# RuihanGao/visual-tactile-synthesis

Hardware: AMD Instinct MI355X
Metric: train_images_per_sec (higher is better)
Workload: dtype f32; 1 GPU; skitG G+D1+D2 train step, 1024x1024 sketch->(RGB,tactile), 4 images/GPU, 64 tactile patches/image, LPIPS/CLIP terms off (no weights offline); global_batch=4, parallelism=dp1, losses_finite=True, hip_graph=True, d2_visualisation_pass=True, train_only=False, full=False

## Files before the change

### include/vts.h

```cpp
#ifndef VTS_H
#define VTS_H

#include <stdint.h>

#ifdef __cplusplus
extern "C" {
#endif

#define VTS_OK 0
#define VTS_ERR_ARG (-1)
#define VTS_ERR_UNSUPPORTED (-2)
#define VTS_ERR_LAUNCH (-3)

#define VTS_ACT_NONE 0
#define VTS_ACT_LRELU 1
#define VTS_ACT_RELU 2
#define VTS_ACT_TANH 3

const char* vts_last_error(void);
const char* vts_last_kernel(void);
int vts_version(void);
int vts_capture_node_count(void* stream, int* nodes, int* kernel_nodes);

typedef struct vts_operand {
  const float* data;
  const float* scale;
  const float* shift;
  int C;
  int64_t nstride;
} vts_operand;

typedef struct vts_conv_desc {
  vts_operand in0, in1;
  int N, IH, IW, OH, OW, Cout;
  int stride, pad, transposed;
  const float* w;
  int ws_co, ws_ci;
  const float* bias;
  float* out;
  int64_t out_nstride;
  int act_in, act_out;
  vts_operand dmask;
  int dmask_act;
  int accumulate;
  float* ws;
  int64_t ws_floats;
  int pad_dx;
} vts_conv_desc;

int64_t vts_conv4x4_ws_floats(const vts_conv_desc* d);

int vts_conv4x4(const vts_conv_desc* d, void* stream);

typedef struct vts_wgrad_desc {
  vts_operand lo0, lo1, hi0, hi1;
  int act_lo, act_hi;
  int N, LH, LW, HH, HW;
  int stride, pad;
  float* dw;
  int accumulate;
  int pad_dx;
  int defer;
} vts_wgrad_desc;

int64_t vts_wgrad4x4_ws_floats(const vts_wgrad_desc* d);
int vts_wgrad4x4(const vts_wgrad_desc* d, float* ws, void* stream);

#define VTS_REDUCE_MAX_SEG 4
typedef struct vts_reduce_job {
  float* dw;
  int64_t nel;
  int accumulate;
  int nseg;
  const float* part[VTS_REDUCE_MAX_SEG];
  int pw[VTS_REDUCE_MAX_SEG];
} vts_reduce_job;
int vts_wgrad_reduce_batch(const vts_reduce_job* jobs , int njobs, void* stream);

int vts_channel_sum(const float* x, int64_t nstride, int N, int C, int HW, float* out, int accumulate,
                    float* ws, int* counters , void* stream);
int64_t vts_channel_sum_ws_floats(int N, int C, int HW);

typedef struct vts_norm_desc {
  const float* x;
  int64_t nstride;
  int N, C, HW;
  int mode;
  float eps, momentum;
  const float* gamma;
  const float* beta;
  float* running_mean;
  float* running_var;
  int64_t* num_batches_tracked;
  float* scale;
  float* shift;
  float* mean_out;
  float* rstd_out;
  int* counters;
  int ngroups;
  int gstart[9];
  float* stat_mean_out;
  float* stat_uvar_out;
  const float* ext_mean;
  const float* ext_uvar;
  int ext_after;
// ... 391 lines not shown
```

### visual-tactile-synthesis_amd/csrc/vts_conv.hip

```cpp
#include "vts_conv_kernel.h"

thread_local int t_stat_spl = 0;

namespace {

__global__ __launch_bounds__(256) void conv_split_epilogue_kernel(const ConvK p, int KS) {
  const int co = blockIdx.y, n = blockIdx.z;
  const int64_t oplane = (int64_t)p.OH * p.OW;
  const int64_t o = (int64_t)blockIdx.x * 256 + threadIdx.x;
  if (o >= oplane) return;
  float v = 0.f;
  for (int ks = 0; ks < KS; ++ks) v += p.part[(((int64_t)ks * p.N + n) * p.Cout + co) * oplane + o];
  v += p.bias ? p.bias[co] : 0.f;
  if (p.act_out == VTS_ACT_TANH) v = tanhf(v);
  if (p.dm) {
    const float dsc = p.dmsc ? p.dmsc[n * p.dmC + co] : 1.f, dsh = p.dmsh ? p.dmsh[n * p.dmC + co] : 0.f;
    v *= vts_act_grad(p.dm[n * p.dmns + co * oplane + o] * dsc + dsh, p.dm_act);
  }
  float* ob = p.out + n * p.ons + co * oplane + o;
  *ob = p.accumulate ? *ob + v : v;
}

struct InStatsOut {
  float *scale, *shift, *mean, *rstd;
  float eps;
};
__global__ __launch_bounds__(256) void conv_split_epilogue_in_kernel(const ConvK p, int KS, const InStatsOut q) {
  __shared__ float red[16];
  const int g = blockIdx.x, n = g / p.Cout, co = g - n * p.Cout;
  const int HW = p.OH * p.OW;
  const float bias = p.bias ? p.bias[co] : 0.f;
  float v[16];
#pragma unroll
  for (int e = 0; e < 16; ++e) {
    const int o = e * 256 + threadIdx.x;
    float a = 0.f;
    if (o < HW) {
      for (int ks = 0; ks < KS; ++ks) a += p.part[(((int64_t)ks * p.N + n) * p.Cout + co) * HW + o];
      a += bias;
      p.out[n * p.ons + (int64_t)co * HW + o] = a;
    }
    v[e] = a;
  }
  const float cnt = (float)HW;
  float s = 0.f;
#pragma unroll
  for (int e = 0; e < 16; ++e) s += v[e];
  const float mean = block_sum(s, red) / cnt;
  float m2 = 0.f;
#pragma unroll
  for (int e = 0; e < 16; ++e) {
    const float d = v[e] - mean;
    if (e * 256 + (int)threadIdx.x < HW) m2 += d * d;
  }
  m2 = block_sum(m2, red);
// ... 18 lines not shown
#pragma unroll
  for (int e = 0; e < 16; ++e) {
    const int o = e * 256 + threadIdx.x;
    float a = 0.f, t = 0.f;
    if (o < HW) {
      for (int ks = 0; ks < KS; ++ks) a += p.part[(((int64_t)ks * p.N + n) * p.Cout + co) * HW + o];
      a += bias;
      t = dmb[o] * dsc + dsh;
      a *= vts_act_grad(t, p.dm_act);
      if (p.accumulate) a += ob[o];
    }
    v[e] = a;
    tn[e] = t;
  }
  float s1 = 0.f, s2 = 0.f;
#pragma unroll
  for (int e = 0; e < 16; ++e) {
    s1 += v[e];
    s2 = fmaf(v[e], tn[e], s2);
  }
  s1 = block_sum(s1, red);
  s2 = block_sum(s2, red);
  const float m1 = s1 / (float)HW, m2 = s2 / (float)HW;
#pragma unroll
  for (int e = 0; e < 16; ++e) {
    const int o = e * 256 + threadIdx.x;
    if (o < HW) ob[o] = dsc * (v[e] - m1 - tn[e] * m2);
  }
}

inline void full_tile(int transposed, int stride, int nr, int& rw, int& mt) {
  static const int T[2][2][5][2] = {
      {{{2, 4}, {1, 4}, {1, 4}, {1, 2}, {1, 2}}, {{2, 4}, {1, 4}, {1, 4}, {1, 2}, {1, 2}}},
      {{{2, 4}, {1, 4}, {1, 4}, {1, 2}, {1, 2}}, {{1, 4}, {1, 2}, {1, 2}, {1, 1}, {1, 1}}}};
  rw = T[transposed][stride - 1][nr - 1][0];
  mt = T[transposed][stride - 1][nr - 1][1];
}

}

extern "C" int64_t vts_conv4x4_ws_floats(const vts_conv_desc* d) {
  if (!d) return 0;
  const int nchunks = (d->in0.C + (d->in1.data ? d->in1.C : 0) + 3) / 4;
  const int ks_max = nchunks / 2 < 1 ? 1 : (nchunks / 2 > 320 ? 320 : nchunks / 2);
  return (int64_t)ks_max * d->N * d->Cout * d->OH * d->OW;
}

struct StatWs {
  float* p;
  int64_t floats;
};
static int conv4x4_impl(const vts_conv_desc* d, void* stream, const vts_norm_desc* nd, int* fused, StatWs sw, bool bsums = false, bool in_bwd_ok = false);
int vts_norm_finalize_partials(const vts_norm_desc* d, const float* part, int spl, hipStream_t st);

extern "C" int vts_conv4x4(const vts_conv_desc* d, void* stream) { return conv4x4_impl(d, stream, nullptr, nullptr, StatWs{nullptr, 0}); }

extern "C" int vts_conv4x4_in(const vts_conv_desc* d, const vts_norm_desc* nd, int* fused, void* stream) {
  VTS_CHECK_ARG(nd && fused && nd->scale && nd->shift && nd->mode == 0, "vts_conv4x4_in: InstanceNorm descriptor with scale / shift outputs required");
  *fused = 0;
  return conv4x4_impl(d, stream, nd, fused, StatWs{nullptr, 0});
}

extern "C" int64_t vts_conv4x4_norm_ws_floats(const vts_conv_desc* d) {
  if (!d) return 0;
  const bool ph4 = d->transposed && d->stride == 2;
  const int GH = ph4 ? (d->OH + 1) / 2 : d->OH, GW = ph4 ? (d->OW + 1) / 2 : d->OW;
  return (int64_t)d->N * d->Cout * 3 * 4 * cdiv(GH, 4) * cdiv(GW, 16);
}

extern "C" int vts_conv4x4_norm(const vts_conv_desc* d, const vts_norm_desc* nd, float* stat_ws, int64_t stat_ws_floats, int* fused, void* stream) {
  VTS_CHECK_ARG(nd && fused && nd->scale && nd->shift && (nd->mode == 0 || nd->mode == 1), "vts_conv4x4_norm: norm descriptor with scale / shift outputs required");
  *fused = 0;
  return conv4x4_impl(d, stream, nd, fused, StatWs{stat_ws, stat_ws_floats});
}

extern "C" int vts_conv4x4_bsums(const vts_conv_desc* d, float* part, int64_t part_floats, int* slots, void* stream) {
  VTS_CHECK_ARG(d && slots && part, "vts_conv4x4_bsums: null pointer");
  const bool in_bwd_ok = *slots == -1;
  *slots = 0;
  int fused = 0;
  const int rc = conv4x4_impl(d, stream, nullptr, &fused, StatWs{part, part_floats}, true, in_bwd_ok);
  if (rc == VTS_OK && fused >= 2) *slots = fused - 2;
  if (rc == VTS_OK && fused == -1) *slots = -1;
  return rc;
}

extern "C" int vts_norm_stats_from_partials(const vts_norm_desc* nd, const float* part, int slots, void* stream) {
  return vts_norm_finalize_partials(nd, part, slots, (hipStream_t)stream);
}

static int dispatch_full(const vts_conv_desc* d, const ConvK& k, int nr, int N, hipStream_t st);

static int conv4x4_impl(const vts_conv_desc* d, void* stream, const vts_norm_desc* nd, int* fused, StatWs sw, bool bsums, bool in_bwd_ok) {
  VTS_CHECK_ARG(d && d->in0.data && d->w && d->out, "vts_conv4x4: null pointer");
  VTS_CHECK_ARG(d->stride == 1 || d->stride == 2, "vts_conv4x4: stride %d unsupported", d->stride);
  VTS_CHECK_ARG(d->Cout >= 1, "vts_conv4x4: Cout %d", d->Cout);
  if (d->Cout > 80) {
    for (int c0 = 0; c0 < d->Cout; c0 += 80) {
      vts_conv_desc g = *d;
      const int64_t oplane = (int64_t)d->OH * d->OW;
      g.Cout = d->Cout - c0 < 80 ? d->Cout - c0 : 80;
      g.w = d->w + (int64_t)c0 * d->ws_co;
      g.bias = d->bias ? d->bias + c0 : nullptr;
      g.out = d->out + c0 * oplane;
      if (d->dmask.data) {
        g.dmask.data = d->dmask.data + c0 * oplane;
        g.dmask.scale = d->dmask.scale ? d->dmask.scale + c0 : nullptr;
        g.dmask.shift = d->dmask.shift ? d->dmask.shift + c0 : nullptr;
      }
      const int rc = conv4x4_impl(&g, stream, nullptr, nullptr, StatWs{nullptr, 0});
      if (rc != VTS_OK) return rc;
    }
    return VTS_OK;
  }
  VTS_CHECK_ARG(d->N >= 1 && d->IH >= 1 && d->IW >= 1 && d->OH >= 1 && d->OW >= 1, "vts_conv4x4: bad shape");
  VTS_CHECK_ARG(d->in0.C >= 1 && d->in1.C >= 0, "vts_conv4x4: bad channel counts");
  VTS_CHECK_ARG(d->OH <= d->IH * d->stride + 16 && d->OW <= d->IW * d->stride + 16 && d->pad >= -8 && d->pad <= 8,
                "vts_conv4x4: output %dx%d / pad %d implausible for input %dx%d s%d", d->OH, d->OW, d->pad, d->IH, d->IW, d->stride);
  VTS_CHECK_ARG(d->pad_dx >= -8 && d->pad_dx <= 8 && !(d->transposed && d->stride == 2 && d->pad_dx != 0), "vts_conv4x4: bad pad_dx %d", d->pad_dx);
  if (d->transposed && d->stride == 2) {
    VTS_CHECK_ARG((d->OH + 2 * d->pad - 4) / d->stride + 1 == d->IH && (d->OW + 2 * d->pad - 4) / d->stride + 1 == d->IW && d->pad >= 0,
                  "vts_conv4x4: transposed output %dx%d inconsistent with input %dx%d s%d p%d", d->OH, d->OW, d->IH,
                  d->IW, d->stride, d->pad);
  }
  {
    const int rh0 = vts_conv_head_try(d, (hipStream_t)stream);
    if (rh0 != VTS_ERR_UNSUPPORTED) return rh0;
    static const int use_small = vts_tune_set("VTS_NO_SMALL") ? 0 : 1;
    if (use_small) {
      const int rc = vts_conv_small_try(d, (hipStream_t)stream);
      if (rc != VTS_ERR_UNSUPPORTED) return rc;
    }
  }
  ConvK k;
  k.s0 = d->in0.data; k.sc0 = d->in0.scale; k.sh0 = d->in0.shift; k.ns0 = d->in0.nstride; k.C0 = d->in0.C;
  k.s1 = d->in1.data; k.sc1 = d->in1.scale; k.sh1 = d->in1.shift; k.ns1 = d->in1.nstride;
  k.C1 = d->in1.data ? d->in1.C : 0;
  k.Cin = k.C0 + k.C1;
  k.IH = d->IH; k.IW = d->IW; k.OH = d->OH; k.OW = d->OW; k.Cout = d->Cout; k.pad = d->pad; k.padx = d->pad + d->pad_dx;
  k.w = d->w; k.ws_co = d->ws_co; k.ws_ci = d->ws_ci; k.bias = d->bias;
  k.out = d->out; k.ons = d->out_nstride;
  k.act_in = d->act_in; k.act_out = d->act_out;
  k.dm = d->dmask.data; k.dmsc = d->dmask.scale; k.dmsh = d->dmask.shift; k.dmns = d->dmask.nstride;
  k.dm_act = d->dmask_act; k.dmC = d->dmask.C;
  k.accumulate = d->accumulate;
  k.N = d->N; k.CG = 1; k.cps = 1 << 30; k.part = nullptr; k.tiles_x = 0; k.stat_part = nullptr; k.stat_spl = 0; k.bsum_part = nullptr;
#ifdef VTS_PROFILING
  static const int ablate = vts_tune("VTS_ABLATE", 0);
  k.ablate = ablate;
  k.trace = nullptr;
#endif
  k.xcd_swizzle = 1;
  static const int direct_epi = vts_tune("VTS_DIRECT_EPI", 1);
  k.direct_epi = direct_epi && (int64_t)d->Cout * d->OH * d->OW * 4 < (int64_t)OOB_OFF && (!d->dmask.data || (int64_t)d->dmask.C * d->OH * d->OW * 4 < (int64_t)OOB_OFF);
  k.ident = vts_ident();
  VTS_CHECK_ARG(k.ident, "vts_conv4x4: could not allocate the identity constants");
  {
    const int64_t wfl = (int64_t)(d->Cout - 1) * d->ws_co + (int64_t)(k.Cin - 1) * d->ws_ci + 16;
    VTS_CHECK_ARG(wfl * 4 < (int64_t)OOB_OFF && (int64_t)d->IH * d->IW * 4 < (int64_t)OOB_OFF, "vts_conv4x4: tensor too large for 30-bit buffer offsets");
    k.wbytes = (int)(wfl * 4);
  }
  k.slope_in = vts_slope(d->act_in);
  k.identity_in = (d->act_in == VTS_ACT_NONE && !d->in0.scale && !d->in0.shift && !(d->in1.data && (d->in1.scale || d->in1.shift))) ? 1 : 0;
  hipStream_t st = (hipStream_t)stream;
  const int nr = (d->Cout + 15) / 16;
  const int N = d->N;
  const bool stats_ok = nd && fused && sw.p && d->act_out == VTS_ACT_NONE && !d->dmask.data && !d->accumulate &&
                        nd->x == d->out && nd->N == N && nd->C == d->Cout && nd->HW == d->OH * d->OW && nd->nstride == d->out_nstride;
  const bool want_stats = stats_ok && k.direct_epi && sw.floats >= vts_conv4x4_norm_ws_floats(d);
  const bool bsums_ok = bsums && fused && sw.p && d->act_out == VTS_ACT_NONE && d->dmask.data;
  const bool want_bsums = bsums_ok && k.direct_epi && sw.floats >= vts_conv4x4_norm_ws_floats(d);
  {
    int spl = 0;
    const int rc = vts_conv_px_try(d, st, stats_ok ? sw.p : nullptr, (!stats_ok && bsums_ok) ? sw.p : nullptr, sw.floats, &spl);
    if (rc != VTS_ERR_UNSUPPORTED) {
      if (rc == VTS_OK && spl > 0) *fused = 2 + spl;
      return rc;
    }
    const int rt = vts_conv_thin_try(d, st);
    if (rt != VTS_ERR_UNSUPPORTED) return rt;
  }
  {
    int rw, mt;
    full_tile(d->transposed, d->stride, nr, rw, mt);
    const bool ph4 = d->transposed && d->stride == 2;
    const int GH = ph4 ? (d->OH + 1) / 2 : d->OH, GW = ph4 ? (d->OW + 1) / 2 : d->OW;
    const int full_wgs = cdiv(GW, 16 * mt) * cdiv(GH, 4 * rw) * N;
    int ck = 4;
    const int nchunks = (k.Cin + 3) / 4;
    static const int small_thr = vts_tune("VTS_SMALL_WGS", 300);
    static const int target_wgs = vts_tune("VTS_TARGET_WGS", 256);
    if (full_wgs < small_thr && (nr > 1 || nchunks >= 8)) {
      const int base = cdiv(GW, 32) * cdiv(GH, 4) * N * nr;
      int KS = target_wgs / base;
      if (KS > nchunks / 2) KS = nchunks / 2;
      if (KS < 1) KS = 1;
      int cps = cdiv(nchunks, KS);
      KS = cdiv(nchunks, cps);
      const int64_t need = (int64_t)KS * N * d->Cout * d->OH * d->OW;
      if (KS > 1 && (!d->ws || d->ws_floats < need)) { KS = 1; cps = nchunks; }
      if (k.Cin >= 32 && cps >= 4 && (cps % 2 == 0 || KS == 1)) { ck = 8; cps = (cps + 1) / 2; }
      k.CG = nr; k.cps = cps; k.part = KS > 1 ? d->ws : nullptr;
      const bool cg_stats = want_stats && KS == 1;
      if (cg_stats) k.stat_part = sw.p;
      const bool cg_bsums = want_bsums && KS == 1;
      if (cg_bsums) k.bsum_part = sw.p;
      int rc;
      if (!d->transposed) rc = d->stride == 2 ? vts_conv_split_m0s2(k, N, st, nr, KS, ck) : vts_conv_split_m0s1(k, N, st, nr, KS, ck);
      else rc = d->stride == 2 ? vts_conv_split_m1s2(k, N, st, nr, KS, ck) : vts_conv_split_m1s1(k, N, st, nr, KS, ck);
      if (rc == VTS_OK && (cg_stats || cg_bsums)) *fused = 2 + t_stat_spl;
      if (rc != VTS_OK || KS == 1) return rc;
      static const int fuse_in = vts_tune("VTS_FUSE_SPLIT_IN", 1);
      if (nd && nd->mode == 0 && fuse_in && (int64_t)d->OH * d->OW <= 4096 && d->act_out == VTS_ACT_NONE && !d->dmask.data && !d->accumulate &&
          nd->x == d->out && nd->N == N && nd->C == d->Cout && nd->HW == d->OH * d->OW && nd->nstride == d->out_nstride) {
        const InStatsOut q{nd->scale, nd->shift, nd->mean_out, nd->rstd_out, nd->eps};
        hipLaunchKernelGGL(conv_split_epilogue_in_kernel, dim3(N * d->Cout), dim3(256), 0, st, k, KS, q);
        VTS_CHECK_LAUNCH("vts_conv4x4 split epilogue + instance norm");
        vts_set_kernel("conv4x4_kernel<%d, %d, 1, 1, 2, %d, false, 0>+ksplit+in", d->transposed ? 1 : 0, d->stride, ck);
        *fused = 1;
        return VTS_OK;
      }
      if (bsums && in_bwd_ok && fused && (int64_t)d->OH * d->OW <= 4096 && d->act_out == VTS_ACT_NONE && d->dmask.data && d->dmask.scale &&
          d->dmask.shift && d->dmask.C == d->Cout) {
        hipLaunchKernelGGL(conv_split_epilogue_inbwd_kernel, dim3(N * d->Cout), dim3(256), 0, st, k, KS);
        VTS_CHECK_LAUNCH("vts_conv4x4 split epilogue + instance norm backward");
        vts_set_kernel("conv4x4_kernel<%d, %d, 1, 1, 2, %d, false, 0>+ksplit+inbwd", d->transposed ? 1 : 0, d->stride, ck);
        *fused = -1;
        return VTS_OK;
      }
      hipLaunchKernelGGL(conv_split_epilogue_kernel, dim3((unsigned)cdiv64((int64_t)d->OH * d->OW, 256), d->Cout, N), dim3(256), 0, st, k, KS);
      VTS_CHECK_LAUNCH("vts_conv4x4 split epilogue");
      return VTS_OK;
    }
  }
  if (want_stats) k.stat_part = sw.p;
  if (want_bsums) k.bsum_part = sw.p;
  const int rc = dispatch_full(d, k, nr, N, st);
  if (rc != VTS_OK || !(want_stats || want_bsums)) return rc;
  *fused = 2 + t_stat_spl;
  return VTS_OK;
}

static int dispatch_full(const vts_conv_desc* d, const ConvK& k, int nr, int N, hipStream_t st) {
  if (!d->transposed) return d->stride == 2 ? vts_conv_full_m0s2(k, nr, N, st) : vts_conv_full_m0s1(k, nr, N, st);
  return d->stride == 2 ? vts_conv_full_m1s2(k, nr, N, st) : vts_conv_full_m1s1(k, nr, N, st);
}
```

### visual-tactile-synthesis_amd/csrc/vts_conv_kernel.h

```cpp
#pragma once
#include <stdio.h>
#include <stdlib.h>
#include <string.h>

#include "vts_internal.h"

struct ConvK {
  const float *s0, *s1, *sc0, *sh0, *sc1, *sh1;
  int64_t ns0, ns1;
  int C0, C1, Cin;
  int IH, IW, OH, OW, Cout, pad, padx;
  const float* w;
  int ws_co, ws_ci;
  const float* bias;
  float* out;
  int64_t ons;
  int act_in, act_out;
  const float *dm, *dmsc, *dmsh;
  int64_t dmns;
  int dm_act, dmC;
  int accumulate;
  int N, CG, cps;
  float* part;
  const float* ident;
  float slope_in;
  int identity_in;
  int wbytes;
  int xcd_swizzle;
  int direct_epi;
  int tiles_x;
  float* stat_part;
  int stat_spl;
  float* bsum_part;
  unsigned rc_gxy, rc_gx, rc_N, rc_CG, rc_gridx;
#ifdef VTS_PROFILING
  int ablate;
  unsigned long long* trace;
#endif
};

#ifdef VTS_PROFILING
#define VTS_ABL(p, bit) ((p).ablate & (bit))
#else
#define VTS_ABL(p, bit) 0
#endif


extern thread_local int t_stat_spl;

int vts_conv_full_m0s1(const ConvK& k, int nr, int N, hipStream_t st);
int vts_conv_full_m0s2(const ConvK& k, int nr, int N, hipStream_t st);
int vts_conv_full_m1s1(const ConvK& k, int nr, int N, hipStream_t st);
int vts_conv_full_m1s2(const ConvK& k, int nr, int N, hipStream_t st);
int vts_conv_split_m0s1(const ConvK& k, int N, hipStream_t st, int CG, int KS, int ck);
int vts_conv_split_m0s2(const ConvK& k, int N, hipStream_t st, int CG, int KS, int ck);
int vts_conv_split_m1s1(const ConvK& k, int N, hipStream_t st, int CG, int KS, int ck);
int vts_conv_split_m1s2(const ConvK& k, int N, hipStream_t st, int CG, int KS, int ck);

namespace {

typedef __amdgpu_buffer_rsrc_t rsrc_t;
constexpr unsigned OOB_OFF = 0x40000000u;
struct TagT { static constexpr bool value = true; };
struct TagF { static constexpr bool value = false; };
__device__ __forceinline__ float ld_buf(const rsrc_t& rs, unsigned voff) {
  return __builtin_bit_cast(float, __builtin_amdgcn_raw_buffer_load_b32(rs, (int)voff, 0, 0));
}

constexpr int conv_min_waves(int mode, int s, int nr, int rw, int mt, bool run) {
  if (run) return rw * mt * ((mode == 1 && s == 2) ? 4 : 1) * nr * 4 <= 48 ? 3 : 2;
  if (mode == 0 && (nr >= 3 || mt >= 4)) return 1;
  const int acc_regs = rw * mt * ((mode == 1 && s == 2) ? 4 : 1) * nr * 4;
  return acc_regs <= 64 ? 4 : (acc_regs <= 96 ? 3 : 2);
}

__host__ inline unsigned conv_recip(unsigned d) { return d <= 1 ? 0u : (unsigned)((0x100000000ull + d - 1) / d); }
__device__ __forceinline__ int fast_div(int n, int d, unsigned rc) {
  if (rc == 0) return n;
  int q = (int)__umulhi((unsigned)n, rc);
  if (q * d > n) --q;
  return q;
}

template <int MODE, int S, int NR, int RW, int MT, int CK, bool RUN, int STATS>
__global__ __launch_bounds__(256, conv_min_waves(MODE, S, NR, RW, MT, RUN)) void conv4x4_kernel(const ConvK p) {
  constexpr int P = (MODE == 1 && S == 2) ? 4 : 1;
  constexpr int TY = 4 * RW, TX = 16 * MT;
  constexpr int PR = MODE == 0 ? (TY - 1) * S + 4 : (S == 2 ? TY + 2 : TY + 3);
  constexpr int PC = MODE == 0 ? (TX - 1) * S + 4 : (S == 2 ? TX + 2 : TX + 3);
  constexpr int PCP = PC + 1;
  constexpr int COP = (NR % 2 == 1) ? NR * 16 : NR * 16 + 16;
  static_assert(CK % 4 == 0 && CK >= 4 && CK <= 16, "staging maps wave w to the input channels w, w + 4, ... of the chunk");
  constexpr int CKW = CK / 4;
  constexpr int REM = PC % 64;
  constexpr int NCM = PC / 64 + ((REM > 16) ? 1 : 0);
  constexpr int PCM = (REM > 16) ? PC : (PC / 64) * 64;
  constexpr int TW = PC - PCM;
  constexpr int NROWS = CK * PR;
  constexpr int NPV = PR * NCM > 0 ? PR * NCM : 1;
  constexpr int NTV = (NROWS * TW + 255) / 256 > 0 ? (NROWS * TW + 255) / 256 : 1;
  constexpr int NWV = CKW * NR;
  constexpr int EC = (P == 4) ? 2 * TX : TX;
  constexpr int EPL = TY * EC + 1;
  constexpr int PATCH_FLOATS = CK * PR * PCP, W_FLOATS = CK * 16 * COP;
  constexpr int OUT_FLOATS = (NR == 1 && RW == 1 && MT == 2) ? 16 * EPL : 0;
  constexpr int LDS_FLOATS = (PATCH_FLOATS + W_FLOATS) > OUT_FLOATS ? (PATCH_FLOATS + W_FLOATS) : OUT_FLOATS;

  __shared__ float lds[LDS_FLOATS];
  __shared__ float lds_stat[STATS ? 4 * NR * 16 * 3 : 1];
  float* lds_patch = lds;
  float* lds_w = lds + PATCH_FLOATS;
// ... 658 lines not shown
  static const char* trace_path = getenv("VTS_CONV_TRACE");
  unsigned long long* trace_dev = nullptr;
  const int64_t trace_wgs = (int64_t)grid.x * grid.y * grid.z;
  if (trace_path) {
    char tag[64];
    snprintf(tag, sizeof tag, "%d,%d,%d,%d,%d", MODE, S, NR, RW, MT);
    const char* want = getenv("VTS_CONV_TRACE_KERNEL");
    if (!want || strcmp(want, tag) == 0) {
      if (hipMalloc(&trace_dev, trace_wgs * 64) != hipSuccess) trace_dev = nullptr;
      if (trace_dev) (void)hipMemsetAsync(trace_dev, 0, trace_wgs * 64, st);
    }
  }
  k.trace = trace_dev;
#endif
  constexpr bool RUNI = (NR <= 2) && CK == 4;
  if (CK != 4) run = 1;
  if (k.stat_part) {
    if (run > 1) hipLaunchKernelGGL((conv4x4_kernel<MODE, S, NR, RW, MT, CK, RUNI, 1>), grid, dim3(256), 0, st, k);
    else hipLaunchKernelGGL((conv4x4_kernel<MODE, S, NR, RW, MT, CK, false, 1>), grid, dim3(256), 0, st, k);
  } else if (k.bsum_part) {
    if (run > 1) hipLaunchKernelGGL((conv4x4_kernel<MODE, S, NR, RW, MT, CK, RUNI, 2>), grid, dim3(256), 0, st, k);
    else hipLaunchKernelGGL((conv4x4_kernel<MODE, S, NR, RW, MT, CK, false, 2>), grid, dim3(256), 0, st, k);
  } else {
    if (run > 1) hipLaunchKernelGGL((conv4x4_kernel<MODE, S, NR, RW, MT, CK, RUNI, 0>), grid, dim3(256), 0, st, k);
    else hipLaunchKernelGGL((conv4x4_kernel<MODE, S, NR, RW, MT, CK, false, 0>), grid, dim3(256), 0, st, k);
  }
  vts_set_kernel("conv4x4_kernel<%d, %d, %d, %d, %d, %d, %s, %s>%s", MODE, S, NR, RW, MT, CK, (run > 1 && NR <= 2) ? "true" : "false",
                 k.stat_part ? "1" : (k.bsum_part ? "2" : "0"), KS > 1 ? "+ksplit" : (CG > 1 ? "+coutsplit" : ""));
  VTS_CHECK_LAUNCH("vts_conv4x4");
#ifdef VTS_PROFILING
  if (trace_dev) {
    (void)hipStreamSynchronize(st);
    unsigned long long* h = (unsigned long long*)malloc(trace_wgs * 64);
    (void)hipMemcpy(h, trace_dev, trace_wgs * 64, hipMemcpyDeviceToHost);
    FILE* f = fopen(trace_path, "a");
    if (f) {
      fprintf(f, "# conv4x4_kernel<%d,%d,%d,%d,%d> run %d grid %u %u %u Cin %d Cout %d OH %d OW %d\n", MODE, S, NR, RW, MT, run, grid.x, grid.y, grid.z, k.Cin, k.Cout, k.OH, k.OW);
      for (int64_t w = 0; w < trace_wgs; ++w) {
        fprintf(f, "%lld %llx", (long long)w, h[w * 8]);
        for (int i = 1; i < 8; ++i) fprintf(f, " %llu", h[w * 8 + i]);
        fprintf(f, "\n");
      }
      fclose(f);
    }
    free(h);
    (void)hipFree(trace_dev);
  }
#endif
  return VTS_OK;
}



}
```

### visual-tactile-synthesis_amd/csrc/vts_conv_m0s1.hip

```cpp
#include "vts_conv_kernel.h"

int vts_conv_full_m0s1(const ConvK& k, int nr, int N, hipStream_t st) {
  switch (nr) {
    case 1: return launch<0, 1, 1, 2, 4, 4>(k, N, st);
    case 2: return launch<0, 1, 2, 1, 4, 4>(k, N, st);
    case 3: return launch<0, 1, 3, 1, 4, 4>(k, N, st);
    case 4: return launch<0, 1, 4, 1, 2, 4>(k, N, st);
    default: return launch<0, 1, 5, 1, 2, 4>(k, N, st);
  }
}

int vts_conv_split_m0s1(const ConvK& k, int N, hipStream_t st, int CG, int KS, int ck) {
  return ck == 8 ? launch<0, 1, 1, 1, 2, 8>(k, N, st, CG, KS) : launch<0, 1, 1, 1, 2, 4>(k, N, st, CG, KS);
}
```

### visual-tactile-synthesis_amd/csrc/vts_conv_m0s2.hip

```cpp
#include "vts_conv_kernel.h"

int vts_conv_full_m0s2(const ConvK& k, int nr, int N, hipStream_t st) {
  switch (nr) {
    case 1: return launch<0, 2, 1, 2, 2, 4>(k, N, st);
    case 2: return vts_prefer_mt3(k, false, 4) ? launch<0, 2, 2, 1, 3, 4>(k, N, st) : launch<0, 2, 2, 1, 4, 4>(k, N, st);
    case 3: return launch<0, 2, 3, 1, 4, 4>(k, N, st);
    case 4: return launch<0, 2, 4, 1, 2, 4>(k, N, st);
    default: return launch<0, 2, 5, 1, 2, 4>(k, N, st);
  }
}

int vts_conv_split_m0s2(const ConvK& k, int N, hipStream_t st, int CG, int KS, int ck) {
  return ck == 8 ? launch<0, 2, 1, 1, 2, 8>(k, N, st, CG, KS) : launch<0, 2, 1, 1, 2, 4>(k, N, st, CG, KS);
}
```

### visual-tactile-synthesis_amd/csrc/vts_conv_m1s1.hip

```cpp
#include "vts_conv_kernel.h"

int vts_conv_full_m1s1(const ConvK& k, int nr, int N, hipStream_t st) {
  switch (nr) {
    case 1: return launch<1, 1, 1, 2, 4, 4>(k, N, st);
    case 2: return vts_prefer_mt3(k, false, 4) ? launch<1, 1, 2, 1, 3, 4>(k, N, st) : launch<1, 1, 2, 1, 4, 4>(k, N, st);
    case 3: return launch<1, 1, 3, 1, 4, 4>(k, N, st);
    case 4: return launch<1, 1, 4, 1, 2, 4>(k, N, st);
    default: return launch<1, 1, 5, 1, 2, 4>(k, N, st);
  }
}

int vts_conv_split_m1s1(const ConvK& k, int N, hipStream_t st, int CG, int KS, int ck) {
  return ck == 8 ? launch<1, 1, 1, 1, 2, 8>(k, N, st, CG, KS) : launch<1, 1, 1, 1, 2, 4>(k, N, st, CG, KS);
}
```

### visual-tactile-synthesis_amd/csrc/vts_conv_m1s2.hip

```cpp
#include "vts_conv_kernel.h"

int vts_conv_full_m1s2(const ConvK& k, int nr, int N, hipStream_t st) {
  switch (nr) {
    case 1: return vts_prefer_mt3(k, true, 4) ? launch<1, 2, 1, 1, 3, 4>(k, N, st) : launch<1, 2, 1, 1, 4, 4>(k, N, st);
    case 2: return launch<1, 2, 2, 1, 2, 4>(k, N, st);
    case 3: return launch<1, 2, 3, 1, 2, 4>(k, N, st);
    case 4: return launch<1, 2, 4, 1, 1, 4>(k, N, st);
    default: return launch<1, 2, 5, 1, 1, 4>(k, N, st);
  }
}

int vts_conv_split_m1s2(const ConvK& k, int N, hipStream_t st, int CG, int KS, int ck) {
  return ck == 8 ? launch<1, 2, 1, 1, 2, 8>(k, N, st, CG, KS) : launch<1, 2, 1, 1, 2, 4>(k, N, st, CG, KS);
}
```

Baseline: 805.4 images/s.

## Add shared-patch conv kernel computing multiple Cout groups per workgroup

Result: no change. 797.9 images/s (-0.9%).

```diff
diff --git a/include/vts.h b/include/vts.h
--- a/include/vts.h
+++ b/include/vts.h
@@ -51,6 +51,8 @@
 int64_t vts_conv4x4_ws_floats(const vts_conv_desc* d);
 
 int vts_conv4x4(const vts_conv_desc* d, void* stream);
+
+int vts_conv4x4_split_member(int member, int ck);
 
 typedef struct vts_wgrad_desc {
   vts_operand lo0, lo1, hi0, hi1;
diff --git a/visual-tactile-synthesis_amd/csrc/vts_conv.hip b/visual-tactile-synthesis_amd/csrc/vts_conv.hip
--- a/visual-tactile-synthesis_amd/csrc/vts_conv.hip
+++ b/visual-tactile-synthesis_amd/csrc/vts_conv.hip
@@ -1,6 +1,7 @@
 #include "vts_conv_kernel.h"
 
 thread_local int t_stat_spl = 0;
+static thread_local int t_split_member = 0, t_split_ck = 0;
 
 namespace {
 
@@ -125,6 +126,19 @@
 };
 static int conv4x4_impl(const vts_conv_desc* d, void* stream, const vts_norm_desc* nd, int* fused, StatWs sw, bool bsums = false, bool in_bwd_ok = false);
 int vts_norm_finalize_partials(const vts_norm_desc* d, const float* part, int spl, hipStream_t st);
+
+extern "C" int vts_conv4x4_split_member(int member, int ck) {
+  VTS_CHECK_ARG(member >= 0 && member <= 3 && (ck == 0 || ck == 4 || ck == 8), "vts_conv4x4_split_member: member %d / ck %d", member, ck);
+  t_split_member = member;
+  t_split_ck = ck;
+  return VTS_OK;
+}
+
+static int split_member_measured(const vts_conv_desc* d, const ConvK& k, int nr, int ck, int tiles) {
+  const int sets = (nr + 2) / 3;
+  if (!d->transposed && d->stride == 2 && !k.identity_in && nr == 5 && ck == 8 && tiles * sets >= 256) return 3;
+  return 1;
+}
 
 extern "C" int vts_conv4x4(const vts_conv_desc* d, void* stream) { return conv4x4_impl(d, stream, nullptr, nullptr, StatWs{nullptr, 0}); }
 
@@ -196,7 +210,10 @@
                   "vts_conv4x4: transposed output %dx%d inconsistent with input %dx%d s%d p%d", d->OH, d->OW, d->IH,
                   d->IW, d->stride, d->pad);
   }
-  {
+  static const int env_member = vts_tune("VTS_SPLIT_MEMBER", 0), env_ck = vts_tune("VTS_SPLIT_CK", 0);
+  const int force = d->Cout > 16 ? (t_split_member ? t_split_member : env_member) : 0;
+  const int force_ck = t_split_member ? t_split_ck : env_ck;
+  if (!force) {
     const int rh0 = vts_conv_head_try(d, (hipStream_t)stream);
     if (rh0 != VTS_ERR_UNSUPPORTED) return rh0;
     static const int use_small = vts_tune_set("VTS_NO_SMALL") ? 0 : 1;
@@ -243,7 +260,7 @@
   const bool want_stats = stats_ok && k.direct_epi && sw.floats >= vts_conv4x4_norm_ws_floats(d);
   const bool bsums_ok = bsums && fused && sw.p && d->act_out == VTS_ACT_NONE && d->dmask.data;
   const bool want_bsums = bsums_ok && k.direct_epi && sw.floats >= vts_conv4x4_norm_ws_floats(d);
-  {
+  if (!force) {
     int spl = 0;
     const int rc = vts_conv_px_try(d, st, stats_ok ? sw.p : nullptr, (!stats_ok && bsums_ok) ? sw.p : nullptr, sw.floats, &spl);
     if (rc != VTS_ERR_UNSUPPORTED) {
@@ -263,23 +280,32 @@
     const int nchunks = (k.Cin + 3) / 4;
     static const int small_thr = vts_tune("VTS_SMALL_WGS", 300);
     static const int target_wgs = vts_tune("VTS_TARGET_WGS", 256);
-    if (full_wgs < small_thr && (nr > 1 || nchunks >= 8)) {
+    if (force || (full_wgs < small_thr && (nr > 1 || nchunks >= 8))) {
       const int base = cdiv(GW, 32) * cdiv(GH, 4) * N * nr;
       int KS = target_wgs / base;
       if (KS > nchunks / 2) KS = nchunks / 2;
-      if (KS < 1) KS = 1;
+      if (KS < 1 || force) KS = 1;
       int cps = cdiv(nchunks, KS);
       KS = cdiv(nchunks, cps);
       const int64_t need = (int64_t)KS * N * d->Cout * d->OH * d->OW;
       if (KS > 1 && (!d->ws || d->ws_floats < need)) { KS = 1; cps = nchunks; }
-      if (k.Cin >= 32 && cps >= 4 && (cps % 2 == 0 || KS == 1)) { ck = 8; cps = (cps + 1) / 2; }
+      if (force && force_ck ? force_ck == 8 : (k.Cin >= 32 && cps >= 4 && (cps % 2 == 0 || KS == 1))) { ck = 8; cps = (cps + 1) / 2; }
       k.CG = nr; k.cps = cps; k.part = KS > 1 ? d->ws : nullptr;
       const bool cg_stats = want_stats && KS == 1;
       if (cg_stats) k.stat_part = sw.p;
       const bool cg_bsums = want_bsums && KS == 1;
       if (cg_bsums) k.bsum_part = sw.p;
       int rc;
-      if (!d->transposed) rc = d->stride == 2 ? vts_conv_split_m0s2(k, N, st, nr, KS, ck) : vts_conv_split_m0s1(k, N, st, nr, KS, ck);
+      const bool can_share = KS == 1 && nr > 1 && k.direct_epi;
+      const int member = force ? force : (can_share ? split_member_measured(d, k, nr, ck, base / nr) : 1);
+      if (member != 1 && !can_share) {
+        vts_set_error("vts_conv4x4: split member %d needs the direct epilogue and no k-split", member);
+        return VTS_ERR_UNSUPPORTED;
+      }
+      if (member == 2 || member == 3) {
+        if (!d->transposed) rc = d->stride == 2 ? vts_conv_share_m0s2(k, N, st, nr, member, ck) : vts_conv_share_m0s1(k, N, st, nr, member, ck);
+        else rc = d->stride == 2 ? vts_conv_share_m1s2(k, N, st, nr, member, ck) : vts_conv_share_m1s1(k, N, st, nr, member, ck);
+      } else if (!d->transposed) rc = d->stride == 2 ? vts_conv_split_m0s2(k, N, st, nr, KS, ck) : vts_conv_split_m0s1(k, N, st, nr, KS, ck);
       else rc = d->stride == 2 ? vts_conv_split_m1s2(k, N, st, nr, KS, ck) : vts_conv_split_m1s1(k, N, st, nr, KS, ck);
       if (rc == VTS_OK && (cg_stats || cg_bsums)) *fused = 2 + t_stat_spl;
       if (rc != VTS_OK || KS == 1) return rc;
diff --git a/visual-tactile-synthesis_amd/csrc/vts_conv_kernel.h b/visual-tactile-synthesis_amd/csrc/vts_conv_kernel.h
--- a/visual-tactile-synthesis_amd/csrc/vts_conv_kernel.h
+++ b/visual-tactile-synthesis_amd/csrc/vts_conv_kernel.h
@@ -57,6 +57,11 @@
 int vts_conv_split_m1s1(const ConvK& k, int N, hipStream_t st, int CG, int KS, int ck);
 int vts_conv_split_m1s2(const ConvK& k, int N, hipStream_t st, int CG, int KS, int ck);
 
+int vts_conv_share_m0s1(const ConvK& k, int N, hipStream_t st, int CG, int G, int ck);
+int vts_conv_share_m0s2(const ConvK& k, int N, hipStream_t st, int CG, int G, int ck);
+int vts_conv_share_m1s1(const ConvK& k, int N, hipStream_t st, int CG, int G, int ck);
+int vts_conv_share_m1s2(const ConvK& k, int N, hipStream_t st, int CG, int G, int ck);
+
 namespace {
 
 typedef __amdgpu_buffer_rsrc_t rsrc_t;
@@ -821,4 +826,504 @@
 
 
 
+template <int MODE, int S, int G, int CK, int STATS>
+__global__ __launch_bounds__(256 * G) void conv4x4_share_kernel(const ConvK p) {
+  constexpr int P = (MODE == 1 && S == 2) ? 4 : 1;
+  constexpr int MT = 2, NW = 4 * G, NT = 256 * G;
+  constexpr int TY = 4, TX = 16 * MT;
+  constexpr int PR = MODE == 0 ? (TY - 1) * S + 4 : (S == 2 ? TY + 2 : TY + 3);
+  constexpr int PC = MODE == 0 ? (TX - 1) * S + 4 : (S == 2 ? TX + 2 : TX + 3);
+  constexpr int PCP = PC + 1;
+  constexpr int NCO = G * 16;
+  constexpr int COP = (G % 2 == 1) ? G * 16 : G * 16 + 16;
+  static_assert(CK == 4 || CK == 8, "weight units: CK / 4 per thread; tails: one wave per chunk channel");
+  static_assert(G == 2 || G == 3, "two or three groups per workgroup");
+  constexpr int REM = PC % 64;
+  constexpr int NCM = PC / 64 + ((REM > 16) ? 1 : 0);
+  constexpr int PCM = (REM > 16) ? PC : (PC / 64) * 64;
+  constexpr int TW = PC - PCM;
+  static_assert(NCM >= 1, "a patch row has at least one 64-column piece");
+  constexpr bool MIXED = NW % CK != 0;
+  static_assert(!MIXED || (CK == 8 && NW == 12), "segment table");
+  constexpr int WPC = MIXED ? 1 : NW / CK;
+  constexpr int NSEG = MIXED ? 2 : 1;
+  constexpr int R1 = MIXED ? (2 * PR + 2) / 3 : (PR + WPC - 1) / WPC;
+  static_assert(MIXED ? (PR - R1 <= R1 && PR > R1) : (WPC - 1) * R1 < PR, "every segment has rows, none more than R1");
+  constexpr int NWV = CK / 4;
+  constexpr int PATCH_FLOATS = CK * PR * PCP, W_FLOATS = CK * 16 * COP;
+
+  __shared__ float lds[PATCH_FLOATS + W_FLOATS];
+  __shared__ float lds_stat[STATS ? NW * 16 * 3 : 1];
+  float* lds_patch = lds;
+  float* lds_w = lds + PATCH_FLOATS;
+
+  const int tid = threadIdx.x, lane = tid & 63;
+  const int wave = __builtin_amdgcn_readfirstlane(tid >> 6);
+  const int wgrp = wave >> 2, wr = wave & 3;
+  const int m16 = lane & 15, kq = lane >> 4;
+  int bx = blockIdx.x, by = blockIdx.y, bz = blockIdx.z;
+  if (p.xcd_swizzle) {
+    const int gx = gridDim.x, gy = gridDim.y, nwg = gx * gy * (int)gridDim.z;
+    const int lin = bx + gx * (by + gy * bz);
+    const int q = nwg >> 3, r = nwg & 7, xcd = lin & 7, idx = lin >> 3;
+    const int lin2 = xcd * q + min(xcd, r) + idx;
+    bz = fast_div(lin2, gx * gy, p.rc_gxy);
+    const int rem = lin2 - bz * (gx * gy);
+    by = fast_div(rem, gx, p.rc_gx);
+    bx = rem - by * gx;
+  }
+  const int cgs = fast_div(bz, p.N, p.rc_N), n = bz - cgs * p.N;
+  const int co0s = cgs * NCO;
+  const int co0 = co0s + wgrp * 16;
+  const bool active = co0 < p.Cout;
+  const int ty0 = by * TY;
+  const int podd = p.pad & 1;
+
+  int iy0;
+  if (MODE == 0) iy0 = ty0 * S - p.pad;
+  else if (S == 2) iy0 = ty0 + (p.pad >> 1) - 1;
+  else iy0 = ty0 + p.pad - 3;
+
+  int aoff[P];
+  if (MODE == 0) {
+    aoff[0] = (wr * S) * PCP + m16 * S + kq;
+  } else if (S == 2) {
+#pragma unroll
+    for (int ph = 0; ph < P; ++ph) {
+      const int dpy = (ph >> 1) & podd, dpx = (ph & 1) & podd;
+      aoff[ph] = (wr + dpy + 1 - (kq >> 1)) * PCP + m16 + dpx + 1 - (kq & 1);
+    }
+  } else {
+    aoff[0] = (wr + 3) * PCP + m16 + 3 - kq;
+  }
+
+  f32x4 acc[MT][P];
+#pragma unroll
+  for (int mt = 0; mt < MT; ++mt)
+#pragma unroll
+    for (int ph = 0; ph < P; ++ph) acc[mt][ph] = (f32x4){0.f, 0.f, 0.f, 0.f};
+
+  const int nchunks = (p.Cin + CK - 1) / CK;
+
+  constexpr int TPR = TW > 0 ? 64 / TW : 1;
+  static_assert(TW == 0 || PR <= TPR, "one tail load covers all patch rows");
+  float pv[NSEG][R1][NCM], tv = 0.f;
+  f32x4 wv[NWV];
+#pragma unroll
+  for (int sg = 0; sg < NSEG; ++sg)
+#pragma unroll
+    for (int r = 0; r < R1; ++r)
+#pragma unroll
+      for (int cm = 0; cm < NCM; ++cm) pv[sg][r][cm] = 0.f;
+#pragma unroll
+  for (int i = 0; i < NWV; ++i) wv[i] = (f32x4){1.f, 1.f, 1.f, 1.f};
+
+  const int iplane = p.IH * p.IW;
+  const float* sb0 = p.s0 + n * p.ns0;
+  const float* sb1 = p.s1 + n * p.ns1;
+  const unsigned row0 = (unsigned)(iy0 * p.IW * 4), rstep = (unsigned)(p.IW * 4);
+  unsigned vo_m[NCM];
+  int colw[NCM];
+  {
+    int ix0;
+    const int tx0 = bx * TX;
+    if (MODE == 0) ix0 = tx0 * S - p.padx;
+    else if (S == 2) ix0 = tx0 + (p.pad >> 1) - 1;
+    else ix0 = tx0 + p.padx - 3;
+#pragma unroll
+    for (int cm = 0; cm < NCM; ++cm) {
+      const int col = cm * 64 + lane, ix = ix0 + col;
+      vo_m[cm] = (col < PCM && ix >= 0 && ix < p.IW) ? (unsigned)ix * 4u : OOB_OFF;
+      colw[cm] = col < PCM ? col : PC;
+    }
+  }
+  unsigned vo_t = OOB_OFF;
+  int dst_t = PC;
+  if (TW > 0) {
+    const int tx0 = bx * TX;
+    const int ix0 = MODE == 0 ? tx0 * S - p.padx : (S == 2 ? tx0 + (p.pad >> 1) - 1 : tx0 + p.padx - 3);
+    const int r_t = lane / (TW > 0 ? TW : 1), c_t = lane - r_t * (TW > 0 ? TW : 1);
+    const int ix = ix0 + PCM + c_t;
+    dst_t = r_t < PR ? r_t * PCP + PCM + c_t : PC;
+    vo_t = (r_t < PR && ix >= 0 && ix < p.IW) ? (unsigned)(r_t * p.IW + ix) * 4u : OOB_OFF;
+  }
+  int sgc[NSEG], sgr0[NSEG], sgn[NSEG];
+  unsigned sgoff[NSEG];
+  if (!MIXED) {
+    const int part = wave / CK;
+    sgc[0] = wave - part * CK;
+    sgr0[0] = part * R1;
+    sgn[0] = min(R1, PR - part * R1);
+  } else {
+#pragma unroll
+    for (int sg = 0; sg < NSEG; ++sg) {
+      sgc[sg] = wave < CK ? wave : 2 * (wave - CK) + sg;
+      sgr0[sg] = wave < CK ? 0 : R1;
+      sgn[sg] = wave < CK ? (sg == 0 ? R1 : 0) : PR - R1;
+    }
+  }
+  float lsc[NSEG], lsh[NSEG], tsc = 1.f, tsh = 0.f;
+  unsigned lnrec[NSEG], tnrec = 0;
+#pragma unroll
+  for (int sg = 0; sg < NSEG; ++sg) {
+    sgoff[sg] = row0 + (unsigned)sgr0[sg] * rstep;
+    lsc[sg] = 1.f;
+    lsh[sg] = 0.f;
+    lnrec[sg] = 0;
+  }
+
+  unsigned wvo[NWV];
+  int wc[NWV], wld[NWV][4];
+#pragma unroll
+  for (int e = 0; e < NWV; ++e) {
+    const int u = tid + e * NT;
+    const int co = u % NCO, rest = u / NCO;
+    const int ky = rest & 3, c = rest >> 2;
+    wc[e] = c;
+    wvo[e] = co0s + co < p.Cout ? (unsigned)((co0s + co) * p.ws_co + c * p.ws_ci + ky * 4) * 4u : OOB_OFF;
+#pragma unroll
+    for (int kx = 0; kx < 4; ++kx) {
+      int slot = ky * 4 + kx;
+      if (MODE == 1 && S == 2) slot = ((((ky + p.pad) & 1) * 2 + ((kx + p.pad) & 1)) * 4) + (ky >> 1) * 2 + (kx >> 1);
+      wld[e][kx] = (c * 16 + slot) * COP + co;
+    }
+  }
+  const rsrc_t wrs = __builtin_amdgcn_make_buffer_rsrc((void*)p.w, 0, p.wbytes, 0x00020000);
+
+  auto opaque_zero = []() {
+    int z = 0;
+    asm volatile("" : "+s"(z));
+    return z;
+  };
+
+  auto channel = [&](int cic, float& sc, float& sh, unsigned& nrec) -> rsrc_t {
+    {
+      const int ccl = min(cic, p.Cin - 1);
+      const bool first = ccl < p.C0;
+      const int cl = first ? ccl : ccl - p.C0;
+      const float* scp = first ? p.sc0 : p.sc1;
+      const float* shp = first ? p.sh0 : p.sh1;
+      const int aidx = n * (first ? p.C0 : p.C1) + cl;
+      const bool hsc = scp != nullptr, hsh = shp != nullptr;
+      sc = (hsc ? scp : p.ident)[hsc ? aidx : 0];
+      sh = (hsh ? shp : p.ident)[hsh ? aidx : 1];
+    }
+    const bool cok = cic < p.Cin;
+    const int cc = cok ? cic : 0;
+    const bool first = cc < p.C0;
+    const float* base = (first ? sb0 : sb1) + (int64_t)(first ? cc : cc - p.C0) * iplane;
+    nrec = cok ? (unsigned)iplane * 4u : 0u;
+    return __builtin_amdgcn_make_buffer_rsrc((void*)base, 0, (int)nrec, 0x00020000);
+  };
+
+  auto load_chunk = [&](int chunk) {
+    const int cbase = chunk * CK;
+#pragma unroll
+    for (int sg = 0; sg < NSEG; ++sg) {
+      if (!MIXED || sgn[sg] > 0) {
+        const rsrc_t rs = channel(cbase + sgc[sg] + opaque_zero(), lsc[sg], lsh[sg], lnrec[sg]);
+#pragma unroll
+        for (int r = 0; r < R1; ++r)
+          if ((!MIXED && WPC == 1) || r < sgn[sg]) {
+#pragma unroll
+            for (int cm = 0; cm < NCM; ++cm) pv[sg][r][cm] = ld_buf(rs, vo_m[cm] + sgoff[sg] + r * rstep);
+          }
+      }
+    }
+    if (TW > 0 && wave < CK) {
+      const rsrc_t rs = channel(cbase + wave + opaque_zero(), tsc, tsh, tnrec);
+      tv = ld_buf(rs, vo_t + row0);
+    }
+    const int wsoff = cbase * p.ws_ci * 4;
+#pragma unroll
+    for (int e = 0; e < NWV; ++e)
+      wv[e] = __builtin_bit_cast(f32x4, __builtin_amdgcn_raw_buffer_load_b128(wrs, (int)(cbase + wc[e] < p.Cin ? wvo[e] : OOB_OFF), wsoff, 0));
+  };
+
+  auto finish = [&](float x, float sc, float sh, bool inside) -> float {
+    const float t = fmaf(x, sc, sh);
+    const float a = fmaxf(t, 0.f) + p.slope_in * fminf(t, 0.f);
+    return inside ? a : 0.f;
+  };
+
+  auto store_patch = [&](auto plain_tag) {
+    constexpr bool PLAIN = decltype(plain_tag)::value;
+#pragma unroll
+    for (int sg = 0; sg < NSEG; ++sg) {
+      float* dst = lds_patch + (sgc[sg] * PR + sgr0[sg]) * PCP;
+#pragma unroll
+      for (int r = 0; r < R1; ++r)
+        if ((!MIXED && WPC == 1) || r < sgn[sg]) {
+#pragma unroll
+          for (int cm = 0; cm < NCM; ++cm) {
+            float v = pv[sg][r][cm];
+            if (!PLAIN) v = finish(v, lsc[sg], lsh[sg], vo_m[cm] + sgoff[sg] + r * rstep < lnrec[sg]);
+            dst[r * PCP + colw[cm]] = v;
+          }
+        }
+    }
+    if (TW > 0 && wave < CK) {
+      float v = tv;
+      if (!PLAIN) v = finish(v, tsc, tsh, vo_t + row0 < tnrec);
+      lds_patch[wave * PR * PCP + dst_t] = v;
+    }
+  };
+
+  auto store_chunk = [&]() {
+    if (p.identity_in) store_patch(TagT());
+    else store_patch(TagF());
+#pragma unroll
+    for (int e = 0; e < NWV; ++e)
+#pragma unroll
+      for (int kx = 0; kx < 4; ++kx) lds_w[wld[e][kx]] = wv[e][kx];
+  };
+
+  if (nchunks > 0) {
+    load_chunk(0);
+    store_chunk();
+  }
+  __syncthreads();
+  for (int chunk = 0; chunk < nchunks; ++chunk) {
+    const bool more = chunk + 1 < nchunks;
+    if (more) load_chunk(chunk + 1);
+    const int cvalid = active ? min(CK, p.Cin - chunk * CK) : 0;
+    {
+      auto rd = [&](int c, int g, float (&av)[MT], float& bv) {
+        const float* pp = lds_patch + c * PR * PCP;
+        bv = lds_w[c * 16 * COP + kq * COP + m16 + wgrp * 16 + g * 4 * COP];
+#pragma unroll
+        for (int mt = 0; mt < MT; ++mt) {
+          if (MODE == 1 && S == 2) av[mt] = pp[aoff[P == 4 ? g : 0] + mt * 16];
+          else if (MODE == 0) av[mt] = pp[aoff[0] + g * PCP + mt * 16 * S];
+          else av[mt] = pp[aoff[0] - g * PCP + mt * 16];
+        }
+      };
+      auto mm = [&](int g, const float (&av)[MT], float bv) {
+#pragma unroll
+        for (int mt = 0; mt < MT; ++mt)
+          acc[mt][P == 4 ? g : 0] = __builtin_amdgcn_mfma_f32_16x16x4f32(av[mt], bv, acc[mt][P == 4 ? g : 0], 0, 0, 0);
+      };
+      float av[4][MT], bv[4];
+      if (cvalid > 0) {
+        rd(0, 0, av[0], bv[0]);
+        rd(0, 1, av[1], bv[1]);
+        rd(0, 2, av[2], bv[2]);
+      }
+      for (int c = 0; c < cvalid; ++c) {
+        const int cn = min(c + 1, CK - 1);
+        rd(c, 3, av[3], bv[3]);
+        __builtin_amdgcn_sched_barrier(0);
+        mm(0, av[0], bv[0]);
+        __builtin_amdgcn_sched_barrier(0);
+        rd(cn, 0, av[0], bv[0]);
+        __builtin_amdgcn_sched_barrier(0);
+        mm(1, av[1], bv[1]);
+        __builtin_amdgcn_sched_barrier(0);
+        rd(cn, 1, av[1], bv[1]);
+        __builtin_amdgcn_sched_barrier(0);
+        mm(2, av[2], bv[2]);
+        __builtin_amdgcn_sched_barrier(0);
+        rd(cn, 2, av[2], bv[2]);
+        __builtin_amdgcn_sched_barrier(0);
+        mm(3, av[3], bv[3]);
+        __builtin_amdgcn_sched_barrier(0);
+      }
+    }
+    __syncthreads();
+    if (more) {
+      store_chunk();
+      __syncthreads();
+    }
+  }
+
+  const int tx0 = bx * TX;
+  const int64_t oplane = (int64_t)p.OH * p.OW;
+  const int onb = (int)((int64_t)p.Cout * oplane * 4);
+  const rsrc_t ors = __builtin_amdgcn_make_buffer_rsrc((void*)(p.out + n * p.ons), 0, onb, 0x00020000);
+  const rsrc_t drs = __builtin_amdgcn_make_buffer_rsrc((void*)(p.dm ? p.dm + n * p.dmns : p.out), 0, p.dm ? (int)((int64_t)p.dmC * oplane * 4) : 0, 0x00020000);
+  const int slot = by * p.tiles_x + bx;
+  if (STATS == 1) {
+    if (active) {
+      float sum = 0.f, sq = 0.f, cnt = 0.f;
+#pragma unroll
+      for (int mt = 0; mt < MT; ++mt)
+#pragma unroll
+        for (int ph = 0; ph < P; ++ph) {
+          const int gy = ty0 + wr, gx = tx0 + mt * 16 + kq * 4;
+          const int y = P == 4 ? gy * 2 + (ph >> 1) : gy, x = P == 4 ? gx * 2 + (ph & 1) : gx;
+          const int nv = y < p.OH ? min(4, P == 4 ? (p.OW - x + 1) >> 1 : p.OW - x) : 0;
+          const f32x4 a = acc[mt][ph];
+#pragma unroll
+          for (int j = 0; j < 4; ++j) {
+            const float v = j < nv ? a[j] : 0.f;
+            sum += v;
+            sq = fmaf(v, v, sq);
+          }
+          cnt += (float)max(nv, 0);
+        }
+      sum += __shfl_xor(sum, 16, 64);
+      sq += __shfl_xor(sq, 16, 64);
+      cnt += __shfl_xor(cnt, 16, 64);
+      sum += __shfl_xor(sum, 32, 64);
+      sq += __shfl_xor(sq, 32, 64);
+      cnt += __shfl_xor(cnt, 32, 64);
+      if (kq == 0) {
+        const float mean = sum / fmaxf(cnt, 1.f);
+        float* q = lds_stat + (wave * 16 + m16) * 3;
+        q[0] = mean;
+        q[1] = fmaxf(sq - sum * mean, 0.f);
+        q[2] = cnt;
+      }
+    }
+    __syncthreads();
+    if (tid < NCO && co0s + tid < p.Cout) {
+      const float* qb = lds_stat + ((tid >> 4) * 64 + (tid & 15)) * 3;
+      float cnt = 0.f, wm = 0.f;
+#pragma unroll
+      for (int w = 0; w < 4; ++w) {
+        const float* q = qb + w * 16 * 3;
+        cnt += q[2];
+        wm = fmaf(q[2], q[0], wm);
+      }
+      const float mean = wm / fmaxf(cnt, 1.f);
+      float m2 = 0.f;
+#pragma unroll
+      for (int w = 0; w < 4; ++w) {
+        const float* q = qb + w * 16 * 3;
+        const float d = q[0] - mean;
+        m2 += q[1] + q[2] * d * d;
+      }
+      const int co = co0s + tid;
+      float* o = p.stat_part + (((int64_t)n * p.Cout + co) * p.stat_spl + slot) * 3;
+      o[0] = mean + (p.bias ? p.bias[co] : 0.f);
+      o[1] = m2;
+      o[2] = cnt;
+    }
+  }
+  float bs1 = 0.f, bs2 = 0.f;
+  auto emit = [&](int co, int y, int x, float bias, float dsc, float dsh, f32x4 v) {
+    const bool ok = co < p.Cout && y < p.OH && x < p.OW;
+    const bool full = ok && x + 4 <= p.OW;
+    const unsigned off = (unsigned)((co * (int)oplane + y * p.OW + x) * 4);
+    const unsigned vo = full ? off : OOB_OFF;
+#pragma unroll
+    for (int j = 0; j < 4; ++j) {
+      float t = v[j] + bias;
+      if (p.act_out == VTS_ACT_TANH) t = tanhf(t);
+      v[j] = t;
+    }
+    const f32x4 base = v;
+    f32x4 tn = {0.f, 0.f, 0.f, 0.f};
+    if (p.dm) {
+      const f32x4 d = __builtin_bit_cast(f32x4, __builtin_amdgcn_raw_buffer_load_b128(drs, (int)vo, 0, 0));
+#pragma unroll
+      for (int j = 0; j < 4; ++j) {
+        tn[j] = d[j] * dsc + dsh;
+        v[j] *= vts_act_grad(tn[j], p.dm_act);
+      }
+    }
+    if (p.accumulate) {
+      const f32x4 q = __builtin_bit_cast(f32x4, __builtin_amdgcn_raw_buffer_load_b128(ors, (int)vo, 0, 0));
+#pragma unroll
+      for (int j = 0; j < 4; ++j) v[j] += q[j];
+    }
+    if (STATS == 2 && full) {
+#pragma unroll
+      for (int j = 0; j < 4; ++j) {
+        bs1 += v[j];
+        bs2 = fmaf(v[j], tn[j], bs2);
+      }
+    }
+    __builtin_amdgcn_raw_buffer_store_b128(__builtin_bit_cast(__attribute__((ext_vector_type(4))) unsigned, v), ors, (int)vo, 0, 0);
+    if (ok && !full) {
+      float* ob = p.out + n * p.ons + co * oplane + (int64_t)y * p.OW + x;
+      const float* db = p.dm ? p.dm + n * p.dmns + co * oplane + (int64_t)y * p.OW + x : nullptr;
+      for (int j = 0; j < p.OW - x; ++j) {
+        float t = base[j];
+        const float tnj = db ? db[j] * dsc + dsh : 0.f;
+        if (db) t *= vts_act_grad(tnj, p.dm_act);
+        const float fin = p.accumulate ? ob[j] + t : t;
+        ob[j] = fin;
+        if (STATS == 2) {
+          bs1 += fin;
+          bs2 = fmaf(fin, tnj, bs2);
+        }
+      }
+    }
+  };
+  if (active) {
+    const int co = co0 + m16;
+    const int coc = min(co, p.Cout - 1);
+    const float bias = p.bias ? p.bias[coc] : 0.f;
+    const float dsc = (p.dm && p.dmsc) ? p.dmsc[n * p.dmC + coc] : 1.f, dsh = (p.dm && p.dmsh) ? p.dmsh[n * p.dmC + coc] : 0.f;
+#pragma unroll
+    for (int mt = 0; mt < MT; ++mt) {
+      const int gy = ty0 + wr, gx = tx0 + mt * 16 + kq * 4;
+      if (P == 1) {
+        emit(co, gy, gx, bias, dsc, dsh, acc[mt][0]);
+      } else {
+#pragma unroll
+        for (int py = 0; py < 2; ++py) {
+          const f32x4 a = acc[mt][P == 4 ? py * 2 : 0], b = acc[mt][P == 4 ? py * 2 + 1 : 0];
+          emit(co, gy * 2 + py, gx * 2, bias, dsc, dsh, (f32x4){a[0], b[0], a[1], b[1]});
+          emit(co, gy * 2 + py, gx * 2 + 4, bias, dsc, dsh, (f32x4){a[2], b[2], a[3], b[3]});
+        }
+      }
+    }
+    if (STATS == 2) {
+      bs1 += __shfl_xor(bs1, 16, 64);
+      bs2 += __shfl_xor(bs2, 16, 64);
+      bs1 += __shfl_xor(bs1, 32, 64);
+      bs2 += __shfl_xor(bs2, 32, 64);
+      if (kq == 0) {
+        float* q = lds_stat + (wave * 16 + m16) * 3;
+        q[0] = bs1;
+        q[1] = bs2;
+      }
+    }
+  }
+  if (STATS == 2) {
+    __syncthreads();
+    if (tid < NCO && co0s + tid < p.Cout) {
+      const float* qb = lds_stat + ((tid >> 4) * 64 + (tid & 15)) * 3;
+      float s1 = 0.f, s2 = 0.f;
+#pragma unroll
+      for (int w = 0; w < 4; ++w) {
+        const float* q = qb + w * 16 * 3;
+        s1 += q[0];
+        s2 += q[1];
+      }
+      float* o = p.bsum_part + (((int64_t)n * p.Cout + co0s + tid) * p.stat_spl + slot) * 2;
+      o[0] = s1;
+      o[1] = s2;
+    }
+  }
 }
+
+template <int MODE, int S, int G, int CK>
+int launch_share(const ConvK& k0, int N, hipStream_t st, int CG) {
+  constexpr int P = (MODE == 1 && S == 2) ? 4 : 1;
+  ConvK k = k0;
+  const int GH = P == 4 ? (k.OH + 1) / 2 : k.OH, GW = P == 4 ? (k.OW + 1) / 2 : k.OW;
+  const int tiles_x = cdiv(GW, 32), tiles_y = cdiv(GH, 4);
+  const int sets = cdiv(CG, G);
+  k.tiles_x = tiles_x;
+  k.stat_spl = tiles_x * tiles_y;
+  t_stat_spl = k.stat_spl;
+  k.CG = sets;
+  dim3 grid(tiles_x, tiles_y, N * sets);
+  k.rc_gxy = conv_recip(grid.x * grid.y); k.rc_gx = k.rc_gridx = conv_recip(grid.x);
+  k.rc_N = conv_recip((unsigned)k.N); k.rc_CG = conv_recip((unsigned)sets);
+  if (k.part || !k.direct_epi) {
+    vts_set_error("vts_conv4x4: the shared-patch member has no LDS epilogue");
+    return VTS_ERR_UNSUPPORTED;
+  }
+  if (k.stat_part) hipLaunchKernelGGL((conv4x4_share_kernel<MODE, S, G, CK, 1>), grid, dim3(256 * G), 0, st, k);
+  else if (k.bsum_part) hipLaunchKernelGGL((conv4x4_share_kernel<MODE, S, G, CK, 2>), grid, dim3(256 * G), 0, st, k);
+  else hipLaunchKernelGGL((conv4x4_share_kernel<MODE, S, G, CK, 0>), grid, dim3(256 * G), 0, st, k);
+  vts_set_kernel("conv4x4_share_kernel<%d, %d, %d, %d, %s>+coutshare%d", MODE, S, G, CK, k.stat_part ? "1" : (k.bsum_part ? "2" : "0"), G);
+  VTS_CHECK_LAUNCH("vts_conv4x4");
+  return VTS_OK;
+}
+
+}
diff --git a/visual-tactile-synthesis_amd/csrc/vts_conv_m0s1.hip b/visual-tactile-synthesis_amd/csrc/vts_conv_m0s1.hip
--- a/visual-tactile-synthesis_amd/csrc/vts_conv_m0s1.hip
+++ b/visual-tactile-synthesis_amd/csrc/vts_conv_m0s1.hip
@@ -13,3 +13,8 @@
 int vts_conv_split_m0s1(const ConvK& k, int N, hipStream_t st, int CG, int KS, int ck) {
   return ck == 8 ? launch<0, 1, 1, 1, 2, 8>(k, N, st, CG, KS) : launch<0, 1, 1, 1, 2, 4>(k, N, st, CG, KS);
 }
+
+int vts_conv_share_m0s1(const ConvK& k, int N, hipStream_t st, int CG, int G, int ck) {
+  if (G == 3) return ck == 8 ? launch_share<0, 1, 3, 8>(k, N, st, CG) : launch_share<0, 1, 3, 4>(k, N, st, CG);
+  return ck == 8 ? launch_share<0, 1, 2, 8>(k, N, st, CG) : launch_share<0, 1, 2, 4>(k, N, st, CG);
+}
diff --git a/visual-tactile-synthesis_amd/csrc/vts_conv_m0s2.hip b/visual-tactile-synthesis_amd/csrc/vts_conv_m0s2.hip
--- a/visual-tactile-synthesis_amd/csrc/vts_conv_m0s2.hip
+++ b/visual-tactile-synthesis_amd/csrc/vts_conv_m0s2.hip
@@ -13,3 +13,8 @@
 int vts_conv_split_m0s2(const ConvK& k, int N, hipStream_t st, int CG, int KS, int ck) {
   return ck == 8 ? launch<0, 2, 1, 1, 2, 8>(k, N, st, CG, KS) : launch<0, 2, 1, 1, 2, 4>(k, N, st, CG, KS);
 }
+
+int vts_conv_share_m0s2(const ConvK& k, int N, hipStream_t st, int CG, int G, int ck) {
+  if (G == 3) return ck == 8 ? launch_share<0, 2, 3, 8>(k, N, st, CG) : launch_share<0, 2, 3, 4>(k, N, st, CG);
+  return ck == 8 ? launch_share<0, 2, 2, 8>(k, N, st, CG) : launch_share<0, 2, 2, 4>(k, N, st, CG);
+}
diff --git a/visual-tactile-synthesis_amd/csrc/vts_conv_m1s1.hip b/visual-tactile-synthesis_amd/csrc/vts_conv_m1s1.hip
--- a/visual-tactile-synthesis_amd/csrc/vts_conv_m1s1.hip
+++ b/visual-tactile-synthesis_amd/csrc/vts_conv_m1s1.hip
@@ -13,3 +13,8 @@
 int vts_conv_split_m1s1(const ConvK& k, int N, hipStream_t st, int CG, int KS, int ck) {
   return ck == 8 ? launch<1, 1, 1, 1, 2, 8>(k, N, st, CG, KS) : launch<1, 1, 1, 1, 2, 4>(k, N, st, CG, KS);
 }
+
+int vts_conv_share_m1s1(const ConvK& k, int N, hipStream_t st, int CG, int G, int ck) {
+  if (G == 3) return ck == 8 ? launch_share<1, 1, 3, 8>(k, N, st, CG) : launch_share<1, 1, 3, 4>(k, N, st, CG);
+  return ck == 8 ? launch_share<1, 1, 2, 8>(k, N, st, CG) : launch_share<1, 1, 2, 4>(k, N, st, CG);
+}
diff --git a/visual-tactile-synthesis_amd/csrc/vts_conv_m1s2.hip b/visual-tactile-synthesis_amd/csrc/vts_conv_m1s2.hip
--- a/visual-tactile-synthesis_amd/csrc/vts_conv_m1s2.hip
+++ b/visual-tactile-synthesis_amd/csrc/vts_conv_m1s2.hip
@@ -13,3 +13,8 @@
 int vts_conv_split_m1s2(const ConvK& k, int N, hipStream_t st, int CG, int KS, int ck) {
   return ck == 8 ? launch<1, 2, 1, 1, 2, 8>(k, N, st, CG, KS) : launch<1, 2, 1, 1, 2, 4>(k, N, st, CG, KS);
 }
+
+int vts_conv_share_m1s2(const ConvK& k, int N, hipStream_t st, int CG, int G, int ck) {
+  if (G == 3) return ck == 8 ? launch_share<1, 2, 3, 8>(k, N, st, CG) : launch_share<1, 2, 3, 4>(k, N, st, CG);
+  return ck == 8 ? launch_share<1, 2, 2, 8>(k, N, st, CG) : launch_share<1, 2, 2, 4>(k, N, st, CG);
+}
```
